# linuxstb/dabtools

Hardware: AMD Instinct MI355X
Metric: ETI frames/s (24 ms each), Mode-I batch, synthetic IQ resident in HBM (higher is better)
Workload: dtype f64 sync / f32 OFDM / u16 ACS / u8 ETI

## Files before the change

### dabtools_amd/csrc/capi_engine.cpp

```cpp
#include <chrono>
#include <memory>
#include <mutex>
#include <new>
#include <string>
#include <vector>

#include "capi_detail.hpp"
#include "engine.hpp"

using namespace dabhip;

struct dabhip_engine {
  Engine eng;
  int nstreams = 0;
  int64_t frames = 0;
  float wall_ms = 0;
  explicit dabhip_engine(int dev, int host_threads = 0, std::vector<int> cpus = {}) : eng(dev, host_threads, std::move(cpus)) {}
  bool has(int stream) const { return stream >= 0 && stream < nstreams; }
};

namespace {

Engine* default_engine()
{
// ... 54 lines not shown
uint32_t dabhip_engine_stream_status(const dabhip_engine* e, int stream) { return e && e->has(stream) ? e->eng.stream_status(stream) : 0xffffffffu; }
int64_t dabhip_engine_eti_read(dabhip_engine* e, int stream, uint8_t* dst, int64_t cap_frames)
{
  if (!e || !dst) { set_error("eti_read: null argument"); return -1; }
  if (!e->has(stream)) { set_error("eti_read: bad stream"); return -1; }
  return e->eng.eti_read(stream, dst, cap_frames);
}
int64_t dabhip_engine_stream_log(dabhip_engine* e, int stream, char* buf, int64_t cap)
{
  if (!e || !e->has(stream)) return -1;
  return hand_over_text(e->eng.take_stream_log(stream), buf, cap);
}
int64_t dabhip_engine_eti_fetch(dabhip_engine* e, uint8_t* dst, int64_t cap_frames)
{
  if (!e || !dst) { set_error("eti_fetch: null argument"); return -1; }
  return e->eng.eti_fetch_async(dst, cap_frames);
}
int dabhip_engine_eti_fetch_wait(dabhip_engine* e)
{
  if (!e) { set_error("eti_fetch_wait: null handle"); return -1; }
  return e->eng.eti_fetch_wait() ? 0 : -1;
}
int64_t dabhip_engine_eti_drain(dabhip_engine* e, dabhip_eti_sink sink, void* user)
{
  if (!e || !sink) { set_error("eti_drain: null argument"); return -1; }
  return drain_eti(e->nstreams, sink, user, true, [e](int b) { return dabhip_engine_eti_count(e, b); },
                   [e](int b, uint8_t* dst, int64_t n) { return dabhip_engine_eti_read(e, b, dst, n); });
}
const void* dabhip_engine_eti_device_ptr(const dabhip_engine* e, int64_t* nframes)
{
  if (!e) return nullptr;
  if (nframes) *nframes = e->frames;
  return e->eng.eti_buffer();
}
int dabhip_engine_demapped_tf(dabhip_engine* e, int stream, int tf, int8_t* fic, int8_t* msc)
{
  if (!e || !fic || !msc) { set_error("demapped_tf: null argument"); return -1; }
  if (!e->has(stream)) { set_error("demapped_tf: bad stream"); return -1; }
  return e->eng.read_demapped_tf(stream, tf, fic, msc) ? 0 : -1;
}
int dabhip_engine_trace(const dabhip_engine* e, int stream, int32_t* ints6, double* ffs, int cap_calls)
{
  if (!e || !ints6 || !e->has(stream)) return -1;
  return e->eng.trace(stream, ints6, ffs, cap_calls);
}
int dabhip_engine_trace_nco(const dabhip_engine* e, int stream, int32_t* nco_hz, int cap_calls)
{
  if (!e || !e->has(stream)) return -1;
  return e->eng.trace_nco(stream, nco_hz, cap_calls);
}
int dabhip_engine_stage_ms(const dabhip_engine* e, const char** names, float* ms, int cap)
{
  if (!e) return -1;
  constexpr int kN = 17;
  static const char* kNames[kN] = {"sync", "fft", "demap", "fic", "control", "gather", "viterbi", "eti", "host_setup", "host_frames", "host_worklist", "wall",
                                   "h2d", "h2d_mbytes", "h2d_pinned_mbytes", "sync_fp64_calls", "sync_spec_calls"};
  const StageTimes& t = e->eng.stage_times();
  const float v[kN] = {t.sync, t.fft, t.demap, t.fic, t.control, t.gather, t.viterbi, t.eti, t.setup, t.frames, t.worklist, e->wall_ms,
                       t.h2d, static_cast<float>(t.h2d_bytes * 1e-6), static_cast<float>(t.h2d_pinned_bytes * 1e-6), t.sync_fp64_calls, t.sync_spec_calls};
  int n = 0;
  for (; n < kN && n < cap; ++n) {
    if (names) names[n] = kNames[n];
    if (ms) ms[n] = v[n];
  }
  return n;
}
int dabhip_engine_set_afc(dabhip_engine* e, int enable) { if (!e) return -1; e->eng.set_afc(enable != 0); return 0; }
int dabhip_engine_set_soft(dabhip_engine* e, int enable) { if (!e) return -1; e->eng.set_soft(enable != 0); return 0; }
int dabhip_engine_set_decoder_forms(dabhip_engine* e, int msc_form, int fic_form)
{
  if (!e) { set_error("set_decoder_forms: null handle"); return -1; }
  return e->eng.set_decoder_forms(msc_form, fic_form) ? 0 : -1;
}
int dabhip_engine_set_soft_lanes(dabhip_engine* e, int enable)
{
  if (!e) { set_error("set_soft_lanes: null handle"); return -1; }
  e->eng.set_soft_lanes(enable != 0);
  return 0;
}
int dabhip_engine_decoder_forms(const dabhip_engine* e, uint32_t* msc_mask, uint32_t* fic_mask)
{
  if (!e) { set_error("decoder_forms: null handle"); return -1; }
  if (msc_mask) *msc_mask = e->eng.msc_forms_ran();
  if (fic_mask) *fic_mask = e->eng.fic_forms_ran();
  return 0;
}
int dabhip_engine_set_subchannels(dabhip_engine* e, const int32_t* ids, int n) { if (!e) return -1; e->eng.set_subchannel_filter(subchannel_mask(ids, n)); return 0; }
int dabhip_engine_set_parity_guard(dabhip_engine* e, int level) { if (!e) return -1; e->eng.set_parity_guard(level); return 0; }
int dabhip_engine_parity_guard_level(const dabhip_engine* e) { return e ? e->eng.parity_guard_level() : -1; }
int dabhip_engine_guard_stats(const dabhip_engine* e, int64_t* flagged, int64_t* decisions)
{
  if (!e) return -1;
  e->eng.guard_stats(flagged, decisions);
  return 0;
}
int dabhip_engine_guard_overflows(const dabhip_engine* e) { return e ? e->eng.guard_overflows() : -1; }
int dabhip_engine_set_guard_list_cap(dabhip_engine* e, uint32_t cap) { if (!e) return -1; e->eng.set_guard_list_cap(cap); return 0; }
int dabhip_engine_set_launch_limits(dabhip_engine* e, const int64_t* limits, int n)
{
  if (!e || !limits || n != kLaunchLimitCount) { set_error("set_launch_limits: bad argument"); return -1; }
  return e->eng.set_launch_limits(limits) ? 0 : -1;
}
int dabhip_engine_launch_report(const dabhip_engine* e, int64_t* out, int cap)
{
  if (!e || !out || cap < 0) { set_error("launch_report: bad argument"); return -1; }
  return report_to_words(e->eng.launch_report(), out, cap);
}
int dabhip_engine_msc_plan(const dabhip_engine* e, int32_t* nsteps, int cap, int64_t* ntiles)
{
  if (!e || cap < 0) { set_error("msc_plan: bad argument"); return -1; }
  return e->eng.msc_plan(nsteps, cap, ntiles);
}
// ... 85 lines not shown
```

### dabtools_amd/csrc/engine.cpp

```cpp
#include "engine_detail.hpp"

#include <cmath>

#include "dab_bits.hpp"
#include "dab_tables.hpp"
#include "placement.hpp"
#include "../../include/dabhip.h"

namespace dabhip {

bool Engine::hard_only(const char* what)
{
  if (soft_bits_ == 0) return true;
  set_error(std::string(what) + ": not available with soft decisions on (dabhip_engine_set_soft): this entry point carries hard bits");
  return false;
}

bool Engine::check(hipError_t e, const char* what)
{
  if (e == hipSuccess) return true;
  set_error(std::string(what) + ": " + hipGetErrorString(e));
  return false;
}
bool Engine::record(hipEvent_t e, hipStream_t s) { return check(hipEventRecord(e, s), "hipEventRecord"); }
bool Engine::elapsed(float* ms, hipEvent_t a, hipEvent_t b) { return check(hipEventElapsedTime(ms, a, b), "hipEventElapsedTime"); }

Engine::Engine(int device, int host_threads, std::vector<int> cpus) : device_(device), host_cpus_(std::move(cpus))
{
  int ndev = 0;
  if (hipGetDeviceCount(&ndev) != hipSuccess || ndev <= 0) { set_error("no HIP device: libdabhip has no CPU fallback"); return; }
  if (device < 0 || device >= ndev) { set_error("device index out of range"); return; }
  if (!check(hipSetDevice(device), "hipSetDevice")) return;
  int prio_low = 0, prio_high = 0;
  (void)hipDeviceGetStreamPriorityRange(&prio_low, &prio_high);
  static const bool side_prio = !(std::getenv("DABHIP_SIDE_PRIORITY") && std::atoi(std::getenv("DABHIP_SIDE_PRIORITY")) == 0);
  if (!check(hipStreamCreate(&stream_), "hipStreamCreate") ||
      !check(side_prio ? hipStreamCreateWithPriority(&copy_stream_, hipStreamDefault, prio_high) : hipStreamCreate(&copy_stream_), "hipStreamCreate"))
    return;
  for (Event* e : {&ev_[0], &ev_[1], &ev_[2], &ev_[3], &ev_upload_, &ev_fic_, &ev_fic_done_, &ev_chain_, &ev_info_, &ev_fibs_, &ev_part0_, &ev_msc_[0], &ev_msc_[1],
                   &ev_msc_[2], &ev_msc_[3], &ev_h2d_[0], &ev_h2d_[1]})
    if (!check(e->create(), "hipEventCreate")) return;
  for (Event& e : stage_ev_)
    if (!check(e.create(false), "hipEventCreate")) return;
  if (!check(hipStreamCreateWithFlags(&d2h_stream_, hipStreamNonBlocking), "hipStreamCreate") || !check(ev_eti_fetch_[0].create(false), "hipEventCreate") ||
      !check(ev_eti_fetch_[1].create(false), "hipEventCreate"))
    return;

  std::vector<double2> tw2048(2048), tw1536(1536);
  std::vector<float2> twf(2048);
  for (int k = 0; k < 2048; ++k) {
    const double a = 2 * M_PI * k / 2048;
    tw2048[k] = make_double2(std::cos(a), std::sin(a));
    if (k % 512 == 0) tw2048[k] = make_double2(k == 0 ? 1.0 : k == 1024 ? -1.0 : 0.0, k == 512 ? 1.0 : k == 1536 ? -1.0 : 0.0);
    twf[k] = make_float2(static_cast<float>(std::cos(a)), static_cast<float>(-std::sin(a)));
  }
  for (int k = 0; k < 1536; ++k) tw1536[k] = make_double2(std::cos(2 * M_PI * k / 1536), std::sin(2 * M_PI * k / 1536));
  std::vector<uint8_t> prs(prs_quarter_turns().begin(), prs_quarter_turns().end());
  std::vector<uint16_t> qpsk(carrier_to_qpsk().begin(), carrier_to_qpsk().end());
  std::vector<uint16_t> crc(256);
  for (int v = 0; v < 256; ++v) {
    const uint8_t b = static_cast<uint8_t>(v);
    crc[v] = crc16_ccitt(&b, 1, 0);
  }
  std::vector<uint16_t> crc_shift(14 * 16);
  for (int i = 0; i < 14; ++i)
    for (int bit = 0; bit < 16; ++bit) {
      if (i == 0) {
        const uint8_t zero = 0;
        crc_shift[bit] = crc16_ccitt(&zero, 1, static_cast<uint16_t>(1u << bit));
      } else {
        uint16_t v = crc_shift[(i - 1) * 16 + bit], y = 0;
        for (int b = 0; b < 16; ++b)
          if ((v >> b) & 1) y ^= crc_shift[(i - 1) * 16 + b];
        crc_shift[i * 16 + bit] = y;
      }
    }
  std::vector<uint32_t> prbs(kMaxCodewordWords), zeros(kMaxCodewordWords, 0u);
  {
    Prbs g;
    for (auto& w : prbs) {
      uint32_t x = 0;
      for (int b = 0; b < 4; ++b) x |= static_cast<uint32_t>(g.next_byte()) << (8 * b);
      w = x;
    }
  }
  if (!d_tw2048_.upload(tw2048, stream_) || !d_tw1536_.upload(tw1536, stream_) || !d_twf_.upload(twf, stream_) ||
      !d_prs_.upload(prs, stream_) || !d_qpsk_.upload(qpsk, stream_) || !d_crc_tab_.upload(crc, stream_) || !d_crc_shift_.upload(crc_shift, stream_) ||
      !d_prbs_.upload(prbs, stream_) || !d_zero_words_.upload(zeros, stream_))
    return;
  if (!check(hipStreamSynchronize(stream_), "table upload")) return;
  const int hw = usable_cpus();
  int nthreads = host_threads > 0 ? std::min(host_threads, 64) : std::max(2, std::min(hw / 2, 24));
  if (const char* env = std::getenv("DABHIP_HOST_THREADS")) nthreads = std::max(1, std::min(64, std::atoi(env)));
// ... 162 lines not shown
      ++report_.fic_prepass;
      GuardArgs ga = soft ? soft_guard_args() : GuardArgs{};
      if (guard && !guard_begin(n, &ga)) return false;
      if (energies && !check(launch_symbol_delta(frame_list(), first, n, 4, d_delta_.get(), kSymbolsPerTf, soft ? kSoftNormC : guard_c_of(guard_rule_level()), stream_), "symbol delta launch"))
        return false;
      if (!check(launch_fic_prepass(soft_bits_, frame_list(), first, n, d_spectra_.get(), ga, stream_), "fic pre-pass launch")) return false;
      if (guard && !guard_finish(true, first, n, 1, 4, false)) return false;
    }
  }
  return record(ev_part0_, stream_);
}

void Engine::control_pass(DecodeRun& run)
{
  (void)hipSetDevice(device_);
  const SegmentLayout& seg = seg_;
  const int nstreams = run.nstreams;
  const uint8_t *const fibs = h_fibs_.data(), *const ok = h_fib_ok_.data();
  const auto t0 = std::chrono::steady_clock::now();
  const bool fresh = planes_fresh_;
  pool_->parallel_for(nstreams, [&](int b) {
    if (fresh) {
      planes_[b] = ControlPlane();
      planes_[b].set_filter(subch_keep_);
    }
    stream_jobs_[b].reserve(static_cast<size_t>(4) * seg.nnew[b]);
    planes_[b].rebase(4 * (carry_[b].prev_used - carry_[b].keep));
    for (int s = seg.tf_base[b] + carry_[b].keep; s < seg.tf_base[b + 1]; ++s)
      planes_[b].on_tf(s - seg.tf_base[b], fibs + static_cast<size_t>(s) * 384, ok + static_cast<size_t>(s) * 12, stream_jobs_[b]);
  });
  std::vector<const ControlPlane*> plane_ptrs(nstreams);
  std::vector<const JobList*> job_ptrs(nstreams);
  total_eti_ = 0;
  for (int b = 0; b < nstreams; ++b) {
    plane_ptrs[b] = &planes_[b];
    job_ptrs[b] = &stream_jobs_[b];
    eti_base_[b] = total_eti_;
    eti_count_[b] = static_cast<int64_t>(stream_jobs_[b].size());
    stream_status_[b] = planes_[b].fault();
    total_eti_ += eti_count_[b];
  }
  planes_fresh_ = false;
  times_.control = ms_since(t0);
  run.mark("control plane done");
  const auto t1 = std::chrono::steady_clock::now();
  run.host_ok = msc_prepare(job_ptrs, plane_ptrs, seg.row_base, seg.fib_base, work_);
  run.mark("work lists built");
  run.host_ok = run.host_ok && msc_upload(work_, copy_stream_) && check(hipEventRecord(ev_upload_, copy_stream_), "work list upload");
  run.mark("work lists queued");
  if (!run.host_ok) run.host_error = dabhip_last_error();
  times_.worklist = ms_since(t1);
}

int64_t Engine::decode_impl(const uint8_t* const* iq, const size_t* nbytes, int nstreams, bool on_device, bool cont, bool full_scan)
{
  if (!ok_) { set_error("engine not initialised (no GPU?)"); return -1; }
  if (nstreams <= 0) { set_error("decode: no streams"); return -1; }
  if (!check(hipSetDevice(device_), "hipSetDevice")) return -1;
  DecodeRun run{nbytes, nstreams, cont, std::chrono::steady_clock::now()};
  times_ = StageTimes{};
  fft_launches_ = fft_tfs_ = 0;
  fft_ms_ = 0;
  guard_new_count();
  guard_decisions_ = 0;
  guard_overflows_ = 0;
  report_ = LaunchReport{};
  last_.pending = false;
  last_.deferred = 0;
  layout_ms_ = 0;
  if (!begin_decode(nstreams, cont)) return -1;
  tii_ms_ = 0;
  tii_ran_ = false;
  if (tii_ && !tii_begin(nstreams, cont)) return -1;
  const SegmentLayout& seg = seg_;
  struct SideStreamGuard {
    hipStream_t s;
    ~SideStreamGuard() { (void)hipStreamSynchronize(s); }
  } side_guard{copy_stream_};
  run.mark("begin_decode done");
  if (!scan_streams(iq, on_device, full_scan, run)) return -1;
  run.mark("scan done");
  times_.setup = scan_setup_ms_;
  for (int b = 0; b < nstreams; ++b) carry_[b].calls_done = std::max(carry_[b].calls_done, static_cast<int>(nbytes[b] / kChunkBytes));
  if (cont && !stage_a(run)) return -1;
  const int ntf = seg.ntf, nslots = seg.tf_base[nstreams], chunk = run.chunk;
  if (ntf == 0) return 0;
  times_.frames = layout_ms_;
  const bool guard = guard_active();
  if (guard) guard_decisions_ += static_cast<int64_t>(ntf) * (kFicBits + kMscBits);
  if (!fic_decode_slots_async(0, nslots, h_fibs_.data(), h_fib_ok_.data(), copy_stream_)) return -1;

  bool gpu_ok = true;
  const int nmsc = seg.nmsc, nchunks = (nmsc + chunk - 1) / chunk;
  while (gpu_ok && static_cast<int>(chunk_ev_.size()) < 3 * nchunks) {
    chunk_ev_.emplace_back();
    gpu_ok = check(chunk_ev_.back().create(), "hipEventCreate");
  }
  gpu_ok = gpu_ok && ofdm_msc_part(0, nmsc, chunk, 0);
  if (tii_) gpu_ok = gpu_ok && tii_launch();
  run.mark("ofdm queued");
  if (!check(hipEventSynchronize(ev_fibs_), "fic decode")) return -1;
  run.mark("fibs on host");
  {
    float part0_ms = 0, fic_ms = 0;
    if (!elapsed(&part0_ms, ev_[3], ev_part0_) || !elapsed(&fic_ms, ev_part0_, ev_fic_done_)) gpu_ok = false;
    times_.fic = fic_ms + (fused_ ? 0.0f : part0_ms);
    if (fused_) times_.fft += part0_ms;
  }

  stream_jobs_.resize(nstreams);
  for (auto& v : stream_jobs_) v.clear();
  host_lane_->post([&]() { control_pass(run); });

  host_lane_->wait();
  if (gpu_ok && run.host_ok)
    gpu_ok = (hipEventQuery(ev_upload_) == hipSuccess || check(hipStreamWaitEvent(stream_, ev_upload_, 0), "work list wait")) && msc_launch_async(work_);
  if (guard && gpu_ok) gpu_ok = guard_download();
  run.mark("all queued");
  const bool drained = check(hipStreamSynchronize(stream_), "decode");
  run.mark("stream drained");
  if (!gpu_ok || !drained) return -1;
  if (!run.host_ok) { set_error(run.host_error); return -1; }
  for (int c = 0; c < nchunks; ++c) {
    float a = 0, d = 0;
    if (!elapsed(&a, chunk_ev_[3 * c], chunk_ev_[3 * c + 1]) || !elapsed(&d, chunk_ev_[3 * c + 1], chunk_ev_[3 * c + 2])) return -1;
    times_.fft += a;
    times_.demap += d;
    fft_ms_ += a;
    fft_launches_ += 1;
    fft_tfs_ += std::min(chunk, nmsc - c * chunk);
  }
  msc_collect();
  if (tii_ran_ && !elapsed(&tii_ms_, ev_tii_[0], ev_tii_[1])) return -1;
  if (!on_device && times_.h2d_bytes > 0 && !elapsed(&times_.h2d, ev_h2d_[0], ev_h2d_[1])) return -1;
  if (guard && !guard_check()) return -1;
  for (int b = 0; b < nstreams; ++b) carry_[b].advance(seg, b);
  last_.chunk = chunk;
  last_.deferred = ntf - nmsc;
  last_.pending = last_.deferred > 0;
  times_.wall = ms_since(run.wall0);
  run.mark("return");
  return total_eti_;
}

int64_t Engine::eti_count(int stream) const { return (stream >= 0 && stream < nstreams_) ? eti_count_[stream] : -1; }
uint32_t Engine::stream_status(int stream) const { return (stream >= 0 && stream < static_cast<int>(stream_status_.size())) ? stream_status_[stream] : 0xffffffffu; }

int64_t Engine::eti_read(int stream, uint8_t* dst, int64_t cap_frames)
{
  if (stream < 0 || stream >= nstreams_) { set_error("eti_read: bad stream"); return -1; }
  const int64_t n = std::min(cap_frames, eti_count_[stream]);
  return read_eti(eti_base_[stream], n, dst) ? n : -1;
}

int64_t Engine::eti_fetch_async(uint8_t* dst, int64_t cap_frames)
{
  if (!dst) { set_error("eti_fetch: null destination"); return -1; }
  if (!check(hipSetDevice(device_), "hipSetDevice")) return -1;
  const uint64_t issued = eti_fetch_issued_.load(), waited = eti_fetch_waited_.load();
  if (issued - waited >= 2) { set_error("eti_fetch: two fetches are outstanding -- eti_fetch_wait first"); return -1; }
  const int64_t n = std::min(cap_frames, total_eti_);
  if (n > 0 && !check(hipMemcpyAsync(dst, d_eti_.get(), static_cast<size_t>(n) * kEtiBytes, hipMemcpyDeviceToHost, d2h_stream_), "eti fetch")) return -1;
  if (!check(hipEventRecord(ev_eti_fetch_[issued & 1], d2h_stream_), "eti fetch event")) return -1;
  eti_fetch_issued_.store(issued + 1);
  return n;
}

bool Engine::eti_fetch_wait()
{
  const uint64_t waited = eti_fetch_waited_.load();
  if (waited == eti_fetch_issued_.load()) return true;
  bool ok = check(hipSetDevice(device_), "hipSetDevice") && check(hipEventSynchronize(ev_eti_fetch_[waited & 1]), "eti fetch");
  if (ok && reap_enabled() && (waited + 1 == eti_fetch_issued_.load() || waited % kReapEvery == kReapEvery - 1)) ok = check(hipStreamSynchronize(d2h_stream_), "eti fetch");
  eti_fetch_waited_.store(waited + 1);
  return ok;
}

const uint8_t* Engine::eti_device(int64_t* nframes) const
{
  if (nframes) *nframes = total_eti_;
  return d_eti_.get();
}

int Engine::trace(int stream, int32_t* ints6, double* ffs, int cap_calls) const
{
// ... 22 lines not shown
```

### dabtools_amd/csrc/engine.hpp

```cpp
#pragma once

#include <hip/hip_runtime.h>

#include <atomic>
#include <chrono>
#include <cstdint>
#include <cstdlib>
#include <map>
#include <memory>
#include <mutex>
#include <new>
#include <string>
#include <utility>
#include <vector>

#include "control_plane.hpp"
#include "decoder_form.hpp"
#include "device_types.hpp"
#include "hip_util.hpp"
#include "launch_limits.hpp"
#include "scan_plan.hpp"
#include "segment_layout.hpp"
#include "thread_pool.hpp"
#include "worklist.hpp"
// ... 11 lines not shown
  PinnedAllocator(const PinnedAllocator<U>&) {}
  T* allocate(size_t n)
  {
    void* p = nullptr;
    if (hipHostMalloc(&p, n * sizeof(T), hipHostMallocDefault) != hipSuccess) throw std::bad_alloc();
    return static_cast<T*>(p);
  }
  void deallocate(T* p, size_t) { (void)hipHostFree(p); }
  template <class U>
  bool operator==(const PinnedAllocator<U>&) const { return true; }
  template <class U>
  bool operator!=(const PinnedAllocator<U>&) const { return false; }
};
template <class T>
using HostList = std::vector<T, PinnedAllocator<T>>;

template <class T>
class PinnedBuffer {
 public:
  PinnedBuffer() = default;
  PinnedBuffer(const PinnedBuffer&) = delete;
  PinnedBuffer& operator=(const PinnedBuffer&) = delete;
  ~PinnedBuffer() { if (p_) (void)hipHostFree(p_); }
  bool resize(size_t n)
  {
    size_ = n;
    if (n <= cap_) return true;
    if (p_) (void)hipHostFree(p_);
    p_ = nullptr;
    cap_ = 0;
    if (hipHostMalloc(reinterpret_cast<void**>(&p_), n * sizeof(T), hipHostMallocDefault) != hipSuccess) {
      p_ = nullptr;
      size_ = 0;
      set_error("hipHostMalloc of " + std::to_string(n * sizeof(T)) + " bytes failed");
      return false;
    }
    cap_ = n;
    return true;
  }
  T* data() const { return p_; }
  size_t size() const { return size_; }
  T& operator[](size_t i) const { return p_[i]; }

 private:
  T* p_ = nullptr;
  size_t cap_ = 0, size_ = 0;
};

struct StageTimes {
  float sync = 0, fft = 0, demap = 0, fic = 0, control = 0, gather = 0, viterbi = 0, eti = 0;
  float setup = 0, frames = 0, worklist = 0, wall = 0;
  float sync_fp64_calls = 0;
  float sync_spec_calls = 0;
  float h2d = 0;
  double h2d_bytes = 0, h2d_pinned_bytes = 0;
};

using DecodeBatch = DecodeBatchT<PinnedAllocator>;
using MscWork = MscWorkT<PinnedAllocator>;

class Engine {
 public:
  explicit Engine(int device, int host_threads = 0, std::vector<int> cpus = {});
  const std::vector<int>& host_cpus() const { return host_cpus_; }
  int numa_node() const { return numa_node_; }
  ~Engine();
  Engine(const Engine&) = delete;
  Engine& operator=(const Engine&) = delete;
  bool ok() const { return ok_; }
  const uint8_t* eti_buffer() const { return d_eti_.get(); }
  void set_afc(bool on) { afc_ = on; }
  void set_fused(bool on) { fused_ = on; }
  void set_demod_all(bool on) { demod_all_ = on; }
  int msc_deferred() const { return last_.deferred; }
  void set_sync_speculation(int mode) { spec_mode_ = mode < 0 ? -1 : (mode > 0 ? 1 : 0); }
  void set_subchannel_filter(uint64_t keep) { subch_keep_ = keep; }
  void set_soft(bool on) { soft_bits_ = on ? 4 : 0; tf_slots_ = 0; msc_rows_ = 0; }
  bool set_decoder_forms(int msc_form, int fic_form);
  void set_soft_lanes(bool on) { knobs_.soft_lanes = on; }
  void clear_forms_ran() { msc_ran_ = 0; fic_ran_ = 0; }
  uint32_t msc_forms_ran() const { return msc_ran_.load(); }
  uint32_t fic_forms_ran() const { return fic_ran_.load(); }
  void set_parity_guard(int level) { guard_level_ = level < 0 ? kDefaultGuardLevel : (level > 2 ? 2 : level); }
  int parity_guard_level() const { return guard_level_; }
  std::string take_stream_log(int stream) { return (stream >= 0 && stream < static_cast<int>(planes_.size())) ? planes_[static_cast<size_t>(stream)].take_log() : std::string(); }
  void guard_stats(int64_t* flagged, int64_t* decisions) const { if (flagged) *flagged = guard_flagged_; if (decisions) *decisions = guard_decisions_; }
  int guard_overflows() const { return guard_overflows_; }
  void set_guard_list_cap(uint32_t cap) { guard_cap_override_ = cap; }
  bool set_launch_limits(const int64_t* v);
  const LaunchLimits& launch_limits() const { return limits_; }
  const LaunchReport& launch_report() const { return report_; }
  void clear_launch_report() { report_ = LaunchReport{}; }
  int msc_plan(int32_t* nsteps, int cap, int64_t* ntiles) const
  {
    const DecodeBatch& b = work_.batch;
    if (ntiles) *ntiles = work_.nframes ? static_cast<int64_t>(b.job_ids.size() / 64) : 0;
    if (work_.nframes == 0) return 0;
    for (size_t g = 0; nsteps && g < b.groups.size() && static_cast<int>(g) < cap; ++g) nsteps[g] = b.groups[g].nsteps;
    return static_cast<int>(b.groups.size());
  }

  int64_t decode(const uint8_t* const* iq, const size_t* nbytes, int nstreams, bool on_device);
  int64_t feed(const uint8_t* const* iq_virtual, const size_t* avail, int nstreams, bool first_segment);
  int64_t stream_need_from(int stream) const;
  int64_t eti_count(int stream) const;
  uint32_t stream_status(int stream) const;
// ... 7 lines not shown
  void fft_stats(int64_t* launches, int64_t* tfs, double* ms) const;
  int fft_roofline(int reps, int64_t* launches, int64_t* tfs, double* ms);

  int stage_ofdm_fft(const uint8_t* frames, int nframes, float* spectra, bool on_device, int reps, float* kernel_ms);
  int stage_demap(const float* spectra, int nframes, uint8_t* fic, uint8_t* msc);
  int stage_fic_decode(const uint8_t* fic, int nframes, uint8_t* fibs, uint8_t* crc_ok);
  int stage_decision_audit(const uint8_t* frames, int nframes, bool on_device, bool guard_on, double* out8, bool fused = false, double* out_extra = nullptr);
  int stage_decision_audit_fused(const uint8_t* frames, int nframes, bool on_device, bool guard_on, double* out8, double* out_extra);
  int viterbi_batch(const uint8_t* symbols, uint8_t* data, int framebits, int n);

  bool reserve_tf_slots(int nslots, int msc_rows = -1);
  bool store_tf_bytes(int slot, const uint8_t* fic_bytes, const uint8_t* msc_bytes);
  bool recycle_tf_slots(int used_slots, int keep_slots);
  bool fic_decode_slots(int first, int n, uint8_t* fibs_host, uint8_t* ok_host);
  bool fic_decode_slots_async(int first, int n, uint8_t* fibs_host, uint8_t* ok_host, hipStream_t copy);
  bool msc_decode(const std::vector<const JobList*>& stream_jobs, const std::vector<const ControlPlane*>& planes,
                  const std::vector<int>& stream_row_base, const std::vector<int>& stream_fib_base)
  {
    return msc_prepare(stream_jobs, planes, stream_row_base, stream_fib_base, work_s3_) && msc_run(work_s3_);
  }
  bool msc_prepare(const std::vector<const JobList*>& stream_jobs, const std::vector<const ControlPlane*>& planes,
                   const std::vector<int>& stream_row_base, const std::vector<int>& stream_fib_base, MscWork& out);
  bool msc_run(MscWork& w);
  bool msc_upload(const MscWork& w, hipStream_t s);
  bool msc_launch(const MscWork& w);
  bool read_eti(int64_t first, int64_t n, uint8_t* dst);
  bool read_demapped_tf(int stream, int tf, int8_t* fic_out, int8_t* msc_out);
  bool scan_one_call(const uint8_t* iq_virtual_base, StreamState* d_state, uint8_t* d_tail, int call, int chunk, CallDesc* out);
  bool demod_one_frame(const uint8_t* iq_virtual_base, const CallDesc& desc, uint8_t* fic_bytes, uint8_t* msc_bytes);
  hipStream_t stream() const { return stream_; }
  int device() const { return device_; }

  void set_tii(bool on) { tii_ = on; }
  bool tii_sums(int stream, uint64_t* T, int* frames);
  bool tii_reset();
  float tii_ms() const { return tii_ms_; }
  int stage_tii(const uint8_t* frames, int nframes, const int32_t* w0, const uint32_t* step, bool on_device, uint64_t* T);

 private:
  bool check(hipError_t e, const char* what);
  bool record(hipEvent_t e, hipStream_t s);
  bool elapsed(float* ms, hipEvent_t a, hipEvent_t b);
  bool hard_only(const char* what);
  struct DecodeRun {
    const size_t* nbytes;
    int nstreams;
    bool cont;
    std::chrono::steady_clock::time_point wall0;
    int chunk = 1;
    bool host_ok = true;
    std::string host_error;
    void mark(const char* what) const;
  };
  int64_t decode_impl(const uint8_t* const* iq, const size_t* nbytes, int nstreams, bool on_device, bool cont, bool full_scan = false);
  bool begin_decode(int nstreams, bool cont);
  bool stage_a(DecodeRun& run);
  void control_pass(DecodeRun& run);
  bool layout_frames(const size_t* nbytes, int nstreams);
  bool layout_and_a(DecodeRun& run) { return layout_frames(run.nbytes, run.nstreams) && (run.cont || stage_a(run)); }
  bool scan_streams(const uint8_t* const* iq, bool on_device, bool full_scan, DecodeRun& run);
  bool scan_begin(const uint8_t* const* iq, bool on_device, bool full_scan, const DecodeRun& run);
  bool scan_chain(bool cont);
  bool scan_fetch();
  bool scan_again(DecodeRun& run);
  SyncArgs sync_args(int nstreams, int max_calls) const;
  bool upload_iq(const uint8_t* const* iq, const size_t* nbytes, int nstreams, const uint8_t** ptrs);
  bool carry_and_reserve(const SegmentLayout& seg);
  struct SmallUpload {
    const void* src;
    void* dst;
    size_t bytes;
    bool pinned;
  };
  static constexpr size_t kSmallUploadBytes = 256 * 1024;
  struct SmallStage {
    PinnedBuffer<uint32_t> words;
    Event done;
    bool armed = false;
  };
  bool upload_small(const SmallUpload* items, int n, hipStream_t s, SmallStage& staging);
  bool launch_decode_batch(const DecodeBatch& b, const uint32_t* bits, const int* d_stream_cif_base, const uint32_t* prbs, uint8_t* out,
                           int record_stride);
  bool msc_launch_async(const MscWork& w);
  void msc_collect();
  bool unpack_tf_slot(int slot, uint8_t* fic_bytes, uint8_t* msc_bytes);

  bool guard_active() const { return guard_level_ > 0 && soft_bits_ == 0 && !afc_; }
  int guard_rule_level() const { return guard_level_ > 0 ? guard_level_ : kDefaultGuardLevel; }
  bool guard_begin(int ntf_in_launch, GuardArgs* out);
  bool guard_finish(bool planar, int first, int n, int sym_a, int sym_b, bool skip_fic);
  bool guard_download();
  bool guard_reserve_counters(int ntf);
  bool guard_check();
  FrameListArgs frame_list() const;
  bool set_frame_list(const uint8_t* d_iq, const CallDesc* descs, int n, int row_lead, bool bit_rows);
  const uint8_t* frames_on_device(const uint8_t* frames, int nframes, bool on_device);
  void guard_new_run() { guard_launches_ = 0; guard_counters_clear_ = false; }
  void guard_new_count() { guard_new_run(); guard_flagged_ = 0; }
  GuardArgs soft_guard_args() const;
  bool fused_parts(int first, int n, int sym_a, int sym_b, int nparts);
  bool ofdm_msc_part(int first, int n, int chunk, int ev_base);
  bool complete_deferred();
  bool tii_tables();
  bool tii_begin(int nstreams, bool cont);
  bool tii_launch();

  bool ok_ = false;
  bool afc_ = false, fused_ = true;
  bool demod_all_ = std::getenv("DABHIP_DEMOD_ALL") != nullptr && std::atoi(std::getenv("DABHIP_DEMOD_ALL")) != 0;
  int guard_level_ = kDefaultGuardLevel;
  uint64_t subch_keep_ = ~0ull;
  int soft_bits_ = 0;
  FormKnobs knobs_;
  int msc_form_ = -1, fic_form_ = -1;
  std::atomic<uint32_t> msc_ran_{0}, fic_ran_{0};
  std::unique_ptr<ThreadPool> pool_;
  std::unique_ptr<AsyncLane> host_lane_;
  int device_ = 0, numa_node_ = -1;
  std::vector<int> host_cpus_;
  hipStream_t stream_ = nullptr, copy_stream_ = nullptr;
  Event ev_[4], ev_upload_, ev_fic_, ev_fic_done_, ev_fibs_, ev_part0_, ev_chain_, ev_info_, ev_msc_[4], ev_h2d_[2];
  hipStream_t d2h_stream_ = nullptr;
  Event ev_eti_fetch_[2];
  std::atomic<uint64_t> eti_fetch_issued_{0}, eti_fetch_waited_{0};
  static constexpr int kStageBufs = 4;
  PinnedBuffer<uint8_t> stage_buf_[kStageBufs];
  Event stage_ev_[kStageBufs];
  bool msc_queued_ = false;
  std::vector<Event> chunk_ev_;

  DeviceBuffer<double2> d_tw2048_, d_tw1536_;
  DeviceBuffer<uint8_t> d_prs_;
  DeviceBuffer<float2> d_twf_;
  DeviceBuffer<uint16_t> d_qpsk_, d_crc_tab_, d_crc_shift_;
  DeviceBuffer<uint32_t> d_prbs_, d_zero_words_;

  DeviceBuffer<uint8_t> d_iq_own_;
  DeviceBuffer<const uint8_t*> d_iq_ptrs_;
  DeviceBuffer<int64_t> d_nbytes_;
  DeviceBuffer<StreamState> d_states_, d_states_prev_;
  DeviceBuffer<uint8_t> d_tail_state_, d_tail_prev_, d_tail_images_;
  DeviceBuffer<int> d_viol_, d_redo_, d_calls_before_;
  PinnedBuffer<int> h_viol_, h_calls_before_;
  SmallStage h_small_fic_, h_small_msc_;
  DeviceBuffer<int2> d_spec_table_;
  DeviceBuffer<int64_t> d_spec_src0_;
  DeviceBuffer<int> d_spec_ctl_;
  PinnedBuffer<int> h_spec_hits_;
  int spec_mode_ = std::getenv("DABHIP_K1_SPEC") ? (std::atoi(std::getenv("DABHIP_K1_SPEC")) > 0 ? 1 : 0) : -1;
  int sync_rescanned_ = 0;
  DeviceBuffer<CallDesc> d_descs_;
  DeviceBuffer<int2> d_info_;
  DeviceBuffer<int2> d_frames_;
  DeviceBuffer<int> d_frame_slot_, d_frame_cif_row_, d_stream_cif_base_;
  DeviceBuffer<float2> d_spectra_;
  DeviceBuffer<uint32_t> d_fic_bits_, d_msc_bits_;
  DeviceBuffer<uint8_t> d_fibs_, d_fib_ok_;
  DeviceBuffer<DecodeJob> d_jobs_;
  DeviceBuffer<WaveGroup> d_groups_;
  DeviceBuffer<int> d_job_ids_;
  DeviceBuffer<CodewordPlan> d_plans_;
  DeviceBuffer<uint4> d_steps_;
  DeviceBuffer<uint32_t> d_grouped_;
  DeviceBuffer<uint2> d_decisions_;
  DeviceBuffer<EtiFrameMeta> d_meta_;
  DeviceBuffer<uint8_t> d_headers_, d_eti_, d_bytes_;
  int tf_slots_ = 0, msc_rows_ = 0;

  std::vector<JobList> stream_jobs_;
  MscWork work_, work_s3_;
  std::vector<ControlPlane> planes_;
  bool planes_fresh_ = false;
  PinnedBuffer<StreamState> h_states_;
  PinnedBuffer<int2> h_frames_;
  PinnedBuffer<const uint8_t*> h_ptrs_;
  PinnedBuffer<int64_t> h_nb_;
  PinnedBuffer<int> h_frame_slot_, h_frame_cif_row_;
  std::vector<StreamCarry> carry_;
  SegmentLayout seg_;
  struct { int chunk = 1, deferred = 0; bool pending = false; } last_;
  std::vector<int> seg_ncalls_, seg_defer_max_;
  std::vector<int> scan_ncalls_;
  DeviceBuffer<float> d_delta_;
  DeviceBuffer<uint4> d_guard_list_;
  DeviceBuffer<uint32_t> d_guard_counter_;
  PinnedBuffer<uint32_t> h_guard_counts_;
  int guard_launches_ = 0;
  bool guard_counters_clear_ = false;
  uint32_t guard_cap_ = 0, guard_cap_override_ = 0;
  LaunchLimits limits_;
  LaunchReport report_;
  std::vector<uint32_t> guard_caps_;
  int64_t guard_flagged_ = 0, guard_decisions_ = 0;
  int guard_overflows_ = 0;
  DeviceBuffer<uint8_t> d_carry_;
  DeviceBuffer<CopyDesc> d_copy_descs_;
  HostList<CopyDesc> carry_out_descs_, carry_in_descs_;

  PlanTable plan_table_;

  bool tii_ = false, tii_ran_ = false;
  int tii_rows_ = 0;
  float tii_ms_ = 0;
// ... 25 lines not shown
```

### dabtools_amd/csrc/engine_scan.cpp

```cpp
#include "engine_detail.hpp"

namespace dabhip {

bool Engine::upload_iq(const uint8_t* const* iq, const size_t* nbytes, int nstreams, const uint8_t** ptrs)
{
  constexpr size_t kStageBytes = size_t(32) << 20, kPiece = size_t(1) << 20;
  if (!record(ev_h2d_[0], stream_)) return false;
  size_t off = 0;
  int next_buf = 0;
  size_t fill = 0;
  size_t fill_dst = 0;
  auto flush = [&]() -> bool {
    if (fill == 0) return true;
    const bool ok = check(hipMemcpyAsync(d_iq_own_.get() + fill_dst, stage_buf_[next_buf].data(), fill, hipMemcpyHostToDevice, stream_), "IQ upload") &&
                    check(hipEventRecord(stage_ev_[next_buf], stream_), "IQ upload");
    next_buf = (next_buf + 1) % kStageBufs;
    fill = 0;
    return ok;
  };
  for (int b = 0; b < nstreams; ++b) {
    uint8_t* const dst = d_iq_own_.get() + off;
    ptrs[b] = dst;
    const size_t n = nbytes[b], padded = (n + 15) & ~size_t(15);
    hipPointerAttribute_t attr;
// ... 4 lines not shown
    if (pinned) {
      if (!flush()) return false;
      times_.h2d_pinned_bytes += static_cast<double>(n);
      if (!check(hipMemcpyAsync(dst, iq[b], n, hipMemcpyDefault, stream_), "IQ upload")) return false;
    } else {
      size_t done = 0;
      while (done < n) {
        if (fill == 0) {
          if (!stage_buf_[next_buf].resize(kStageBytes)) return false;
          if (!check(hipEventSynchronize(stage_ev_[next_buf]), "IQ staging")) return false;
          fill_dst = off + done;
        }
        const size_t take = std::min(n - done, kStageBytes - fill);
        const uint8_t* src = iq[b] + done;
        uint8_t* stage = stage_buf_[next_buf].data() + fill;
        const int pieces = static_cast<int>((take + kPiece - 1) / kPiece);
        pool_->parallel_for(pieces, [&](int i) {
          const size_t a = static_cast<size_t>(i) * kPiece;
          std::memcpy(stage + a, src + a, std::min(kPiece, take - a));
        });
        fill += take;
        done += take;
        if (fill == kStageBytes && !flush()) return false;
      }
      if (padded != n && !flush()) return false;
    }
    off += padded;
  }
  if (!flush()) return false;
  if (!record(ev_h2d_[1], stream_)) return false;
  return true;
}

SyncArgs Engine::sync_args(int nstreams, int max_calls) const
{
  return SyncArgs{d_iq_ptrs_.get(), d_nbytes_.get(), d_states_.get(), d_descs_.get(), d_info_.get(), nstreams, max_calls, d_tw2048_.get(), d_tw1536_.get(), d_prs_.get()};
}

bool Engine::scan_streams(const uint8_t* const* iq, bool on_device, bool full_scan, DecodeRun& run)
{
  const int nstreams = run.nstreams;
  if (!scan_begin(iq, on_device, full_scan, run)) return false;
  const ScanPlan& p = scan_;
  sync_rescanned_ = 0;
  if (!record(ev_[0], stream_)) return false;
  if (!p.split) {
    SyncScanOpts o;
    o.afc = afc_ ? 1 : 0;
    o.tails = SyncTails{d_tail_state_.get(), d_tail_state_.get(), d_tail_images_.get(), kChunkBytes};
    if (!check(launch_sync_scan(sync_args(nstreams, p.max_calls), o, stream_), "sync scan launch")) return false;
  } else if (!scan_chain(run.cont)) {
    return false;
  }
  if (!record(ev_[1], stream_)) return false;
  if (p.split && (!check(hipEventSynchronize(ev_info_), "call info") || !layout_and_a(run))) return false;
  if (!scan_fetch()) return false;
  if (!p.split && !layout_and_a(run)) return false;
  if (p.split && !scan_again(run)) return false;
  if (!check(hipStreamWaitEvent(copy_stream_, ev_[1], 0), "desc download") ||
      !check(hipMemcpyAsync(h_descs_.data(), d_descs_.get(), p.ndesc * sizeof(CallDesc), hipMemcpyDeviceToHost, copy_stream_), "desc download"))
    return false;
  if (!elapsed(&times_.sync, ev_[0], ev_[1])) return false;
  for (int b = 0; b < nstreams; ++b)
    if (h_states_[b].overflow) { set_error("sync scan: stale-tail bookkeeping overflow (more than kMaxSeg nested short reads)"); return false; }
  return true;
}

bool Engine::scan_begin(const uint8_t* const* iq, bool on_device, bool full_scan, const DecodeRun& run)
{
  const auto wall0 = std::chrono::steady_clock::now();
  const int nstreams = run.nstreams;
  if (!h_ptrs_.resize(nstreams) || !h_nb_.resize(nstreams) || !h_calls_before_.resize(nstreams)) return false;
  const uint8_t** const ptrs = h_ptrs_.data();
  scan_ncalls_.resize(nstreams);
  size_t total = 0;
  for (int b = 0; b < nstreams; ++b) {
    h_nb_[b] = static_cast<int64_t>(run.nbytes[b]);
    scan_ncalls_[b] = static_cast<int>(run.nbytes[b] / kChunkBytes);
    h_calls_before_[b] = carry_[b].calls_done;
    total += (run.nbytes[b] + 15) & ~size_t(15);
  }
  static const ScanKnobs knobs = ScanKnobs::from_env();
  const ScanPlan p = plan_scan(nstreams, scan_ncalls_.data(), h_calls_before_.data(), afc_, full_scan, run.cont, spec_mode_, knobs);
  if (!h_descs_.resize(p.ndesc) || !h_info_.resize(p.ndesc)) return false;
  scan_ = p;
  if (on_device) {
    for (int b = 0; b < nstreams; ++b) ptrs[b] = iq[b];
  } else {
    if (!d_iq_own_.reserve(total) || !upload_iq(iq, run.nbytes, nstreams, ptrs)) return false;
  }
  if (!h_states_.resize(nstreams)) return false;
  StreamState* const states = h_states_.data();
  if (!run.cont) std::fill(states, states + nstreams, initial_state());
  static_assert(sizeof(CallDesc) % 16 == 0, "cleared in 16-byte pieces");
  if (!d_states_.reserve(nstreams) || !d_iq_ptrs_.reserve(nstreams) || !d_nbytes_.reserve(nstreams) || !d_descs_.reserve(p.ndesc) || !d_info_.reserve(p.ndesc + 1)) return false;
  if (!d_tail_state_.reserve(static_cast<size_t>(nstreams) * kTailBytes) || !d_tail_images_.reserve(p.ndesc * kTailBytes) ||
      (p.split && !d_tail_prev_.reserve(static_cast<size_t>(nstreams) * kTailBytes)))
    return false;
  if (p.ahead && (!d_spec_table_.reserve(static_cast<size_t>(nstreams) * p.nspec * p.nhyp) || !d_spec_src0_.reserve(static_cast<size_t>(nstreams) * p.nspec) ||
                  !d_spec_ctl_.reserve(nstreams + 1) || !h_spec_hits_.resize(1)))
    return false;
  if (p.split && (!h_viol_.resize(nstreams + 1) || !d_viol_.reserve(nstreams + 1) || !d_states_prev_.reserve(nstreams) || !d_calls_before_.reserve(nstreams))) return false;
  ScanSetupArgs a{};
  a.h_states = run.cont ? nullptr : states;
  a.h_ptrs = ptrs;
  a.h_nbytes = h_nb_.data();
  a.h_calls_before = p.split ? h_calls_before_.data() : nullptr;
  a.states = d_states_.get();
  a.states_prev = p.split ? d_states_prev_.get() : nullptr;
  a.iq_ptrs = d_iq_ptrs_.get();
  a.nbytes = d_nbytes_.get();
  a.calls_before = p.split ? d_calls_before_.get() : nullptr;
  a.viol = p.split ? d_viol_.get() : nullptr;
  a.descs = reinterpret_cast<uint4*>(d_descs_.get());
  a.desc_vec = p.ndesc * (sizeof(CallDesc) / 16);
  a.info = reinterpret_cast<uint4*>(d_info_.get());
  a.info_vec = (p.ndesc + 1) / 2;
  a.nstreams = nstreams;
  a.tail_state = d_tail_state_.get();
  a.tail_state_prev = p.split ? d_tail_prev_.get() : nullptr;
  if (!check(launch_scan_setup(a, stream_), "scan setup launch")) return false;
  scan_setup_ms_ = ms_since(wall0);
  return true;
}

bool Engine::scan_chain(bool cont)
{
  const ScanPlan& p = scan_;
  const SyncArgs a = sync_args(nstreams_, p.max_calls);
  SyncScanOpts o;
  o.chain_only = true;
  o.tails = SyncTails{d_tail_state_.get(), d_tail_state_.get(), d_tail_images_.get(), kChunkBytes};
  auto chain = [&]() { return check(launch_sync_scan(a, o, stream_), "sync chain launch"); };
  if (p.ahead) {
    SpecArgs& sp = o.spec;
    sp.table = d_spec_table_.get();
    sp.src0 = d_spec_src0_.get();
    sp.ctl = d_spec_ctl_.get();
    sp.nspec = p.nspec;
    sp.nstreams = nstreams_;
    sp.nhyp = p.nhyp;
    sp.call_limit = p.first_limit;
    sp.record_base = 1;
    if (!chain()) return false;
    sp.record_base = 0;
    sp.lookup = 1;
    for (int r = 0; r < p.passes; ++r) {
      sp.call_limit = p.pass_limit(r);
      if (!check(launch_sync_ahead(a, sp, stream_), "sync look-ahead launch") || !chain()) return false;
    }
  } else if (!chain()) {
    return false;
  }
  return check(hipEventRecord(ev_chain_, stream_), "chain event") && check(hipStreamWaitEvent(copy_stream_, ev_chain_, 0), "chain event") &&
         check(hipMemcpyAsync(h_info_.data(), d_info_.get(), p.ndesc * sizeof(int2), hipMemcpyDeviceToHost, copy_stream_), "call info download") &&
         check(hipEventRecord(ev_info_, copy_stream_), "call info event") &&
         check(launch_sync_verify(a, d_calls_before_.get(), d_viol_.get(), false, stream_), "sync verify launch") &&
         check(launch_sync_verify(a, d_calls_before_.get(), d_viol_.get(), true, stream_), "sync carry launch");
}

bool Engine::scan_fetch()
{
  const ScanPlan& p = scan_;
  const int nstreams = nstreams_;
  StreamState* const states = h_states_.data();
  ++report_.fetches;
  report_.fetch_form = p.result_words <= static_cast<size_t>(limits_.fetch_words) ? kFetchKernel : kFetchCopyEngine;
  if (report_.fetch_form == kFetchKernel) {
    HostWordsArgs hw{};
    int k = 0;
    auto add = [&](const void* src, void* dst, size_t n) { hw.set(k++, src, dst, n); };
    if (p.split) add(d_viol_.get(), h_viol_.data(), nstreams + 1);
    if (p.ahead) add(d_spec_ctl_.get() + nstreams, h_spec_hits_.data(), 1);
    add(d_info_.get(), h_info_.data(), p.ndesc * 2);
    add(d_states_.get(), states, static_cast<size_t>(nstreams) * (sizeof(StreamState) / 4));
    return check(hipStreamWaitEvent(copy_stream_, ev_[1], 0), "scan event") && check(launch_host_words(hw, copy_stream_), "scan results download") &&
           check(hipStreamSynchronize(copy_stream_), "sync scan");
  }
  return check(hipStreamWaitEvent(copy_stream_, ev_[1], 0), "scan event") &&
         (!p.split || check(hipMemcpyAsync(h_viol_.data(), d_viol_.get(), (nstreams + 1) * sizeof(int), hipMemcpyDeviceToHost, copy_stream_), "violation download")) &&
         (!p.ahead || check(hipMemcpyAsync(h_spec_hits_.data(), d_spec_ctl_.get() + nstreams, sizeof(int), hipMemcpyDeviceToHost, copy_stream_), "look-ahead hits download")) &&
         check(hipMemcpyAsync(h_info_.data(), d_info_.get(), p.ndesc * sizeof(int2), hipMemcpyDeviceToHost, copy_stream_), "call info download") &&
         check(hipMemcpyAsync(states, d_states_.get(), nstreams * sizeof(StreamState), hipMemcpyDeviceToHost, copy_stream_), "state download") &&
         check(hipStreamSynchronize(copy_stream_), "sync scan");
}

bool Engine::scan_again(DecodeRun& run)
{
  const int nstreams = nstreams_;
  std::vector<int> redo;
  for (int b = 0; b < nstreams; ++b)
    if (h_viol_[b] != 0x7f7f7f7f) redo.push_back(b);
  sync_rescanned_ = static_cast<int>(redo.size());
  times_.sync_fp64_calls = static_cast<float>(h_viol_[nstreams]);
  times_.sync_spec_calls = scan_.ahead ? static_cast<float>(h_spec_hits_[0]) : 0.0f;
  if (redo.empty()) return true;
  guard_new_run();
  SyncScanOpts o;
  o.states_in = d_states_prev_.get();
  o.tails = SyncTails{d_tail_prev_.get(), d_tail_state_.get(), d_tail_images_.get(), kChunkBytes};
  if (!check(hipStreamSynchronize(stream_), "before the rescan") || !d_redo_.upload(redo, stream_)) return false;
  o.stream_list = d_redo_.get();
  return check(launch_sync_scan(sync_args(sync_rescanned_, scan_.max_calls), o, stream_), "sync rescan launch") && record(ev_[1], stream_) && scan_fetch() &&
         layout_and_a(run);
}

}
```

### dabtools_amd/csrc/scan_plan.hpp

```cpp
#pragma once

#include <algorithm>
#include <cstddef>
#include <cstdlib>

#include "device_types.hpp"

namespace dabhip {

struct ScanKnobs {
  int hypotheses = 33, spec_max_streams = 4;
  static int odd_window(int v) { return std::max(3, std::min(63, v | 1)); }
  static ScanKnobs from_env()
  {
    ScanKnobs k;
    if (const char* e = std::getenv("DABHIP_K1_HYP")) k.hypotheses = std::atoi(e);
    if (const char* e = std::getenv("DABHIP_K1_SPEC_MAX_STREAMS")) k.spec_max_streams = std::atoi(e);
    return k;
  }
};

struct ScanPlan {
  int max_calls = 1;
  size_t ndesc = 0;
  bool split = false;
  bool ahead = false;
  int nspec = 0;
  int nhyp = 0, passes = 0;
  int first_limit = 0;
  size_t result_words = 0;
  int pass_limit(int r) const { return r + 1 < passes ? nspec : -1; }
};

inline ScanPlan plan_scan(int nstreams, const int* ncalls, const int* calls_done, bool afc, bool full_scan, bool cont, int spec_mode, const ScanKnobs& knobs)
{
  constexpr int kAheadMinCalls = 16, kAheadForcedMaxStreams = 512;
  ScanPlan p;
  for (int b = 0; b < nstreams; ++b) p.max_calls = std::max(p.max_calls, ncalls[b] - calls_done[b]);
  p.ndesc = static_cast<size_t>(nstreams) * p.max_calls;
  p.split = !(afc || full_scan);
  p.ahead = p.split && spec_mode != 0 &&
            (spec_mode > 0 ? nstreams <= kAheadForcedMaxStreams : (nstreams <= std::max(0, std::min(512, knobs.spec_max_streams)) && p.max_calls >= kAheadMinCalls));
  p.nspec = std::min(p.max_calls, std::min(4096, std::max(64, (1 << 20) / nstreams)));
  p.nhyp = ScanKnobs::odd_window(knobs.hypotheses);
  p.passes = std::min(16, (p.max_calls + p.nspec - 1) / p.nspec);
  p.first_limit = cont ? 0 : 7;
  p.result_words = (p.split ? nstreams + 1 : 0) + (p.ahead ? 1 : 0) + p.ndesc * 2 + static_cast<size_t>(nstreams) * (sizeof(StreamState) / 4);
  return p;
}

}
```

Before: 4.882 million.

## Defer sync verification off the critical path and redecode on violation

When the scan is split, not look-ahead, not continuous and OFDM is fused, the fp64 sync verify and carry kernels move to the copy stream. The host proceeds to layout, OFDM and FIC decode without waiting for the verdict, which it checks after the FIBs arrive. If any stream violated, the engine drains both streams and reruns the whole decode with inline verification. This removes a host-device synchronisation and the serial verify from the critical path, at the cost of a full redecode when speculation fails and extra stream contention.

```diff
diff --git a/dabtools_amd/csrc/capi_engine.cpp b/dabtools_amd/csrc/capi_engine.cpp
--- a/dabtools_amd/csrc/capi_engine.cpp
+++ b/dabtools_amd/csrc/capi_engine.cpp
@@ -130,12 +130,13 @@
 int dabhip_engine_stage_ms(const dabhip_engine* e, const char** names, float* ms, int cap)
 {
   if (!e) return -1;
-  constexpr int kN = 17;
+  constexpr int kN = 20;
   static const char* kNames[kN] = {"sync", "fft", "demap", "fic", "control", "gather", "viterbi", "eti", "host_setup", "host_frames", "host_worklist", "wall",
-                                   "h2d", "h2d_mbytes", "h2d_pinned_mbytes", "sync_fp64_calls", "sync_spec_calls"};
+                                   "h2d", "h2d_mbytes", "h2d_pinned_mbytes", "sync_fp64_calls", "sync_spec_calls", "sync_verify", "sync_verify_deferred", "sync_redecoded"};
   const StageTimes& t = e->eng.stage_times();
   const float v[kN] = {t.sync, t.fft, t.demap, t.fic, t.control, t.gather, t.viterbi, t.eti, t.setup, t.frames, t.worklist, e->wall_ms,
-                       t.h2d, static_cast<float>(t.h2d_bytes * 1e-6), static_cast<float>(t.h2d_pinned_bytes * 1e-6), t.sync_fp64_calls, t.sync_spec_calls};
+                       t.h2d, static_cast<float>(t.h2d_bytes * 1e-6), static_cast<float>(t.h2d_pinned_bytes * 1e-6), t.sync_fp64_calls, t.sync_spec_calls, t.sync_verify,
+                       t.sync_verify_deferred, t.sync_redecoded};
   int n = 0;
   for (; n < kN && n < cap; ++n) {
     if (names) names[n] = kNames[n];
diff --git a/dabtools_amd/csrc/engine.cpp b/dabtools_amd/csrc/engine.cpp
--- a/dabtools_amd/csrc/engine.cpp
+++ b/dabtools_amd/csrc/engine.cpp
@@ -37,8 +37,8 @@
   if (!check(hipStreamCreate(&stream_), "hipStreamCreate") ||
       !check(side_prio ? hipStreamCreateWithPriority(&copy_stream_, hipStreamDefault, prio_high) : hipStreamCreate(&copy_stream_), "hipStreamCreate"))
     return;
-  for (Event* e : {&ev_[0], &ev_[1], &ev_[2], &ev_[3], &ev_upload_, &ev_fic_, &ev_fic_done_, &ev_chain_, &ev_info_, &ev_fibs_, &ev_part0_, &ev_msc_[0], &ev_msc_[1],
-                   &ev_msc_[2], &ev_msc_[3], &ev_h2d_[0], &ev_h2d_[1]})
+  for (Event* e : {&ev_[0], &ev_[1], &ev_[2], &ev_[3], &ev_upload_, &ev_fic_, &ev_fic_done_, &ev_chain_, &ev_info_, &ev_verify_done_, &ev_fibs_, &ev_part0_, &ev_msc_[0],
+                   &ev_msc_[1], &ev_msc_[2], &ev_msc_[3], &ev_h2d_[0], &ev_h2d_[1]})
     if (!check(e->create(), "hipEventCreate")) return;
   for (Event& e : stage_ev_)
     if (!check(e.create(false), "hipEventCreate")) return;
@@ -307,13 +307,16 @@
   times_.worklist = ms_since(t1);
 }
 
-int64_t Engine::decode_impl(const uint8_t* const* iq, const size_t* nbytes, int nstreams, bool on_device, bool cont, bool full_scan)
-{
+int64_t Engine::decode_impl(const uint8_t* const* iq, const size_t* nbytes, int nstreams, bool on_device, bool cont, bool full_scan, bool verify_inline)
+{
+  verify_inline_once_ = verify_inline;
+  verify_deferred_ = false;
   if (!ok_) { set_error("engine not initialised (no GPU?)"); return -1; }
   if (nstreams <= 0) { set_error("decode: no streams"); return -1; }
   if (!check(hipSetDevice(device_), "hipSetDevice")) return -1;
   DecodeRun run{nbytes, nstreams, cont, std::chrono::steady_clock::now()};
   times_ = StageTimes{};
+  times_.sync_redecoded = verify_inline ? 1.0f : 0.0f;
   fft_launches_ = fft_tfs_ = 0;
   fft_ms_ = 0;
   guard_new_count();
@@ -339,7 +342,11 @@
   for (int b = 0; b < nstreams; ++b) carry_[b].calls_done = std::max(carry_[b].calls_done, static_cast<int>(nbytes[b] / kChunkBytes));
   if (cont && !stage_a(run)) return -1;
   const int ntf = seg.ntf, nslots = seg.tf_base[nstreams], chunk = run.chunk;
-  if (ntf == 0) return 0;
+  if (ntf == 0) {
+    bool violated = false;
+    if (verify_deferred_ && (!check(hipStreamSynchronize(copy_stream_), "sync scan") || !scan_verdict(&violated))) return -1;
+    return 0;
+  }
   times_.frames = layout_ms_;
   const bool guard = guard_active();
   if (guard) guard_decisions_ += static_cast<int64_t>(ntf) * (kFicBits + kMscBits);
@@ -352,10 +359,19 @@
     gpu_ok = check(chunk_ev_.back().create(), "hipEventCreate");
   }
   gpu_ok = gpu_ok && ofdm_msc_part(0, nmsc, chunk, 0);
-  if (tii_) gpu_ok = gpu_ok && tii_launch();
+  if (tii_) gpu_ok = gpu_ok && (!verify_deferred_ || check(hipStreamWaitEvent(stream_, ev_verify_done_, 0), "verification wait")) && tii_launch();
   run.mark("ofdm queued");
   if (!check(hipEventSynchronize(ev_fibs_), "fic decode")) return -1;
   run.mark("fibs on host");
+  if (verify_deferred_) {
+    bool violated = false;
+    const bool verdict_ok = scan_verdict(&violated);
+    if (!verdict_ok || violated) {
+      const bool drained = check(hipStreamSynchronize(stream_), "decode") && check(hipStreamSynchronize(copy_stream_), "decode");
+      if (!verdict_ok || !drained || !gpu_ok) return -1;
+      return decode_impl(iq, nbytes, nstreams, on_device, cont, full_scan, true);
+    }
+  }
   {
     float part0_ms = 0, fic_ms = 0;
     if (!elapsed(&part0_ms, ev_[3], ev_part0_) || !elapsed(&fic_ms, ev_part0_, ev_fic_done_)) gpu_ok = false;
@@ -386,6 +402,7 @@
     fft_tfs_ += std::min(chunk, nmsc - c * chunk);
   }
   msc_collect();
+  if (verify_deferred_ && !elapsed(&times_.sync_verify, ev_info_, ev_verify_done_)) return -1;
   if (tii_ran_ && !elapsed(&tii_ms_, ev_tii_[0], ev_tii_[1])) return -1;
   if (!on_device && times_.h2d_bytes > 0 && !elapsed(&times_.h2d, ev_h2d_[0], ev_h2d_[1])) return -1;
   if (guard && !guard_check()) return -1;
diff --git a/dabtools_amd/csrc/engine.hpp b/dabtools_amd/csrc/engine.hpp
--- a/dabtools_amd/csrc/engine.hpp
+++ b/dabtools_amd/csrc/engine.hpp
@@ -87,6 +87,9 @@
   float setup = 0, frames = 0, worklist = 0, wall = 0;
   float sync_fp64_calls = 0;
   float sync_spec_calls = 0;
+  float sync_verify = 0;
+  float sync_verify_deferred = 0;
+  float sync_redecoded = 0;
   float h2d = 0;
   double h2d_bytes = 0, h2d_pinned_bytes = 0;
 };
@@ -200,7 +203,7 @@
     std::string host_error;
     void mark(const char* what) const;
   };
-  int64_t decode_impl(const uint8_t* const* iq, const size_t* nbytes, int nstreams, bool on_device, bool cont, bool full_scan = false);
+  int64_t decode_impl(const uint8_t* const* iq, const size_t* nbytes, int nstreams, bool on_device, bool cont, bool full_scan = false, bool verify_inline = false);
   bool begin_decode(int nstreams, bool cont);
   bool stage_a(DecodeRun& run);
   void control_pass(DecodeRun& run);
@@ -209,7 +212,8 @@
   bool scan_streams(const uint8_t* const* iq, bool on_device, bool full_scan, DecodeRun& run);
   bool scan_begin(const uint8_t* const* iq, bool on_device, bool full_scan, const DecodeRun& run);
   bool scan_chain(bool cont);
-  bool scan_fetch();
+  bool scan_fetch(bool deferred = false);
+  bool scan_verdict(bool* violated);
   bool scan_again(DecodeRun& run);
   SyncArgs sync_args(int nstreams, int max_calls) const;
   bool upload_iq(const uint8_t* const* iq, const size_t* nbytes, int nstreams, const uint8_t** ptrs);
@@ -297,6 +301,10 @@
   PinnedBuffer<int> h_spec_hits_;
   int spec_mode_ = std::getenv("DABHIP_K1_SPEC") ? (std::atoi(std::getenv("DABHIP_K1_SPEC")) > 0 ? 1 : 0) : -1;
   int sync_rescanned_ = 0;
+  const bool verify_inline_ = std::getenv("DABHIP_VERIFY_INLINE") != nullptr && std::atoi(std::getenv("DABHIP_VERIFY_INLINE")) != 0;
+  bool verify_deferred_ = false;
+  bool verify_inline_once_ = false;
+  Event ev_verify_done_;
   DeviceBuffer<CallDesc> d_descs_;
   DeviceBuffer<int2> d_info_;
   DeviceBuffer<int2> d_frames_;
diff --git a/dabtools_amd/csrc/engine_scan.cpp b/dabtools_amd/csrc/engine_scan.cpp
--- a/dabtools_amd/csrc/engine_scan.cpp
+++ b/dabtools_amd/csrc/engine_scan.cpp
@@ -80,6 +80,12 @@
   } else if (!scan_chain(run.cont)) {
     return false;
   }
+  if (verify_deferred_) {
+    if (!check(hipEventSynchronize(ev_info_), "call info") || !layout_and_a(run) || !scan_fetch(true) ||
+        !check(hipMemcpyAsync(h_descs_.data(), d_descs_.get(), p.ndesc * sizeof(CallDesc), hipMemcpyDeviceToHost, copy_stream_), "desc download"))
+      return false;
+    return elapsed(&times_.sync, ev_[0], ev_chain_);
+  }
   if (!record(ev_[1], stream_)) return false;
   if (p.split && (!check(hipEventSynchronize(ev_info_), "call info") || !layout_and_a(run))) return false;
   if (!scan_fetch()) return false;
@@ -89,6 +95,7 @@
       !check(hipMemcpyAsync(h_descs_.data(), d_descs_.get(), p.ndesc * sizeof(CallDesc), hipMemcpyDeviceToHost, copy_stream_), "desc download"))
     return false;
   if (!elapsed(&times_.sync, ev_[0], ev_[1])) return false;
+  if (p.split && !elapsed(&times_.sync_verify, ev_chain_, ev_[1])) return false;
   for (int b = 0; b < nstreams; ++b)
     if (h_states_[b].overflow) { set_error("sync scan: stale-tail bookkeeping overflow (more than kMaxSeg nested short reads)"); return false; }
   return true;
@@ -112,6 +119,8 @@
   const ScanPlan p = plan_scan(nstreams, scan_ncalls_.data(), h_calls_before_.data(), afc_, full_scan, run.cont, spec_mode_, knobs);
   if (!h_descs_.resize(p.ndesc) || !h_info_.resize(p.ndesc)) return false;
   scan_ = p;
+  verify_deferred_ = verify_deferred(p, run.cont, fused_, verify_inline_ || verify_inline_once_);
+  times_.sync_verify_deferred = verify_deferred_ ? 1.0f : 0.0f;
   if (on_device) {
     for (int b = 0; b < nstreams; ++b) ptrs[b] = iq[b];
   } else {
@@ -180,18 +189,22 @@
   } else if (!chain()) {
     return false;
   }
+  const hipStream_t vs = verify_deferred_ ? copy_stream_ : stream_;
   return check(hipEventRecord(ev_chain_, stream_), "chain event") && check(hipStreamWaitEvent(copy_stream_, ev_chain_, 0), "chain event") &&
          check(hipMemcpyAsync(h_info_.data(), d_info_.get(), p.ndesc * sizeof(int2), hipMemcpyDeviceToHost, copy_stream_), "call info download") &&
          check(hipEventRecord(ev_info_, copy_stream_), "call info event") &&
-         check(launch_sync_verify(a, d_calls_before_.get(), d_viol_.get(), false, stream_), "sync verify launch") &&
-         check(launch_sync_verify(a, d_calls_before_.get(), d_viol_.get(), true, stream_), "sync carry launch");
-}
-
-bool Engine::scan_fetch()
+         check(launch_sync_verify(a, d_calls_before_.get(), d_viol_.get(), false, vs), "sync verify launch") &&
+         check(launch_sync_verify(a, d_calls_before_.get(), d_viol_.get(), true, vs), "sync carry launch") &&
+         (!verify_deferred_ || check(hipEventRecord(ev_verify_done_, vs), "verification event"));
+}
+
+bool Engine::scan_fetch(bool deferred)
 {
   const ScanPlan& p = scan_;
   const int nstreams = nstreams_;
   StreamState* const states = h_states_.data();
+  auto behind_scan = [&]() { return deferred || check(hipStreamWaitEvent(copy_stream_, ev_[1], 0), "scan event"); };
+  auto awaited = [&]() { return deferred || check(hipStreamSynchronize(copy_stream_), "sync scan"); };
   ++report_.fetches;
   report_.fetch_form = p.result_words <= static_cast<size_t>(limits_.fetch_words) ? kFetchKernel : kFetchCopyEngine;
   if (report_.fetch_form == kFetchKernel) {
@@ -202,15 +215,26 @@
     if (p.ahead) add(d_spec_ctl_.get() + nstreams, h_spec_hits_.data(), 1);
     add(d_info_.get(), h_info_.data(), p.ndesc * 2);
     add(d_states_.get(), states, static_cast<size_t>(nstreams) * (sizeof(StreamState) / 4));
-    return check(hipStreamWaitEvent(copy_stream_, ev_[1], 0), "scan event") && check(launch_host_words(hw, copy_stream_), "scan results download") &&
-           check(hipStreamSynchronize(copy_stream_), "sync scan");
-  }
-  return check(hipStreamWaitEvent(copy_stream_, ev_[1], 0), "scan event") &&
+    return behind_scan() && check(launch_host_words(hw, copy_stream_), "scan results download") && awaited();
+  }
+  return behind_scan() &&
          (!p.split || check(hipMemcpyAsync(h_viol_.data(), d_viol_.get(), (nstreams + 1) * sizeof(int), hipMemcpyDeviceToHost, copy_stream_), "violation download")) &&
          (!p.ahead || check(hipMemcpyAsync(h_spec_hits_.data(), d_spec_ctl_.get() + nstreams, sizeof(int), hipMemcpyDeviceToHost, copy_stream_), "look-ahead hits download")) &&
          check(hipMemcpyAsync(h_info_.data(), d_info_.get(), p.ndesc * sizeof(int2), hipMemcpyDeviceToHost, copy_stream_), "call info download") &&
          check(hipMemcpyAsync(states, d_states_.get(), nstreams * sizeof(StreamState), hipMemcpyDeviceToHost, copy_stream_), "state download") &&
-         check(hipStreamSynchronize(copy_stream_), "sync scan");
+         awaited();
+}
+
+bool Engine::scan_verdict(bool* violated)
+{
+  const int nstreams = nstreams_;
+  *violated = false;
+  for (int b = 0; b < nstreams; ++b) *violated = *violated || h_viol_[b] != 0x7f7f7f7f;
+  times_.sync_fp64_calls = static_cast<float>(h_viol_[nstreams]);
+  times_.sync_spec_calls = 0.0f;
+  for (int b = 0; b < nstreams; ++b)
+    if (h_states_[b].overflow) { set_error("sync scan: stale-tail bookkeeping overflow (more than kMaxSeg nested short reads)"); return false; }
+  return true;
 }
 
 bool Engine::scan_again(DecodeRun& run)
diff --git a/dabtools_amd/csrc/scan_plan.hpp b/dabtools_amd/csrc/scan_plan.hpp
--- a/dabtools_amd/csrc/scan_plan.hpp
+++ b/dabtools_amd/csrc/scan_plan.hpp
@@ -49,4 +49,9 @@
   return p;
 }
 
+inline bool verify_deferred(const ScanPlan& p, bool cont, bool fused_ofdm, bool forced_inline)
+{
+  return p.split && !p.ahead && !cont && fused_ofdm && !forced_inline;
 }
+
+}
```

Measured after the change: 4.939 million, median of 6. +1.2%, better.
